# qianlim/CAPE

Hardware: AMD Instinct MI355X
Metric: meshes/sec fwd+bwd, CAPE-affineconv nz64 @ batch 16, 1/2/4/8 MI355X (higher is better)
Workload: dtype f32

## Files before the change

cape_amd/_lib.py:

```python
import ctypes as C
import os

import torch

_HERE = os.path.dirname(os.path.abspath(__file__))
LIB_PATH = os.path.join(_HERE, "libcape_hip.so")

MAX_SRC = 8
ACT = {"none": 0, "leaky": 1, "relu": 2, "tanh": 3}
BIAS_NONE, BIAS_CHANNEL, BIAS_VERTEX = 0, 1, 2


class CapeSrc(C.Structure):
    _fields_ = [
        ("x", C.c_void_p), ("x_sample_stride", C.c_int64), ("ldx", C.c_int32), ("C", C.c_int32),
        ("w", C.c_void_p), ("w_rs", C.c_int64), ("w_cs", C.c_int64),
        ("w2", C.c_void_p), ("w2_rs", C.c_int64), ("w2_cs", C.c_int64),
    ]


class CapeCondLayer(C.Structure):
    _fields_ = [("w", C.c_void_p), ("w_aff", C.c_void_p), ("coef", C.c_void_p), ("dcoef", C.c_void_p),
                ("gw", C.c_void_p), ("gw_aff", C.c_void_p), ("K", C.c_int32), ("F", C.c_int32)]

# ... 68 lines not shown
    "cape_gconv_fwd": (C.c_int, [_SRCP, _i32, _p, _i64, _i32, _i32, _i32, _i32, _p, _i32, _i32, _p,
                                 C.POINTER(CapeRank), _i32, _p]),
    "cape_gconv_fwd_plan": (C.c_int, [_SRCP, _i32, _i32, _i32, _i32, C.POINTER(_i32)]),
    "cape_gconv_fwd_h2": (C.c_int, [_SRCP, _i32, _p, _i64, _i32, _i32, _i32, _i32, _p, _i32, _i32, _p,
                                    C.POINTER(CapeRank), _i32, C.POINTER(CapeH2), _p]),
    "cape_gconv_fwd_plan_h2": (C.c_int, [_SRCP, _i32, _i32, _i32, _i32, C.POINTER(CapeH2), C.POINTER(_i32)]),
    "cape_gconv_dw_stage_h2": (C.c_int, [_SRCP, _i32, _p, _i64, _i32, _p, C.c_uint32, _i32, _i32, _i32, _i32, _p, _i64, _i32,
                                         C.POINTER(CapeH2Dw), _p]),
    "cape_gconv_dw_plan_h2": (C.c_int, [_SRCP, _i32, _p, _i64, _i32, _p, C.c_uint32, _i32, _i32, _i32, C.POINTER(CapeH2Dw),
                                        C.POINTER(_i32)]),
    "cape_rowmax": (C.c_int, [_p, _i64, _i32, _i32, _i32, _i32, _p, _i32, _p]),
    "cape_weight_pieces_blocks": (C.c_int, [C.c_void_p, _i32, C.POINTER(_i32), C.POINTER(_i32)]),
    "cape_weight_pieces": (C.c_int, [_p, _i32, _p, _i32, _p, _i32, _p]),
    "cape_rowscale_reduce_workspace_bytes": (_i64, [_i32, _i32, _i32, _i32]),
    "cape_rowscale_reduce": (C.c_int, [_p, _i64, _i32, _p, _i32, _i32, _i32, _i32, _p, _p, _i64, _p]),
    "cape_gconv_dw_workspace_bytes": (_i64, [_SRCP, _i32, _i32, _i32, _i32]),
    "cape_gconv_dw": (C.c_int, [_SRCP, _i32, _p, _i64, _i32, _p, C.c_uint32, _i32, _i32, _i32, _i32, _p, _i64, _p]),
    "cape_gconv_dw_stage": (C.c_int, [_SRCP, _i32, _p, _i64, _i32, _p, C.c_uint32, _i32, _i32, _i32, _i32, _p, _i64, _i32, _p]),
    "cape_condnet_fwd": (C.c_int, [_p, _i32, _p, _i32, _p, _p, _p, _p, _p, _p, _p, _p, _p, _i32, _i32, _i32, _i32, _i32, _i32, _p]),
    "cape_condnet_bwd": (C.c_int, [_p, _i32, _p, _i32, _p, _p, _p, _i32, _p, _i32, _p, _p, _p, _p, _p, _p, _i32, _i32, _i32, _i32, _i32, _i32, _p]),
    "cape_gconv_dw_reduce_batch": (C.c_int, [C.c_void_p, _i32, _p]),
    "cape_gconv_dw_batch": (C.c_int, [C.c_void_p, _i32, _p]),
    "cape_gconv_dw_batch_plan": (C.c_int, [C.c_void_p, _i32, C.POINTER(_i32), _i32, C.POINTER(_i32)]),
    "cape_gconv_dw_plan": (C.c_int, [_SRCP, _i32, _p, _i64, _i32, _p, C.c_uint32, _i32, _i32, _i32, C.POINTER(_i32)]),
    "cape_gconv_fwd_bf16": (C.c_int, [_SRCP, _i32, _p, _i64, _i32, _i32, _i32, _i32, _p, _i32, _i32, _p,
                                      C.POINTER(CapeRank), _i32, _p]),
    "cape_gconv_fwd_plan_bf16": (C.c_int, [_SRCP, _i32, _i32, _i32, _i32, C.POINTER(_i32)]),
    "cape_gconv_dw_bf16": (C.c_int, [_SRCP, _i32, _p, _i64, _i32, _p, C.c_uint32, _i32, _i32, _i32, _i32, _p, _i64, _p]),
    "cape_gconv_dw_stage_bf16": (C.c_int, [_SRCP, _i32, _p, _i64, _i32, _p, C.c_uint32, _i32, _i32, _i32, _i32, _p, _i64, _i32, _p]),
    "cape_gconv_dw_plan_bf16": (C.c_int, [_SRCP, _i32, _p, _i64, _i32, _p, C.c_uint32, _i32, _i32, _i32, C.POINTER(_i32)]),
    "cape_bwd_prep_workspace_bytes": (_i64, [_i32, _i32, _i32, _i32]),
    "cape_bwd_prep": (C.c_int, [_p, _i64, _i32, _p, _i64, _i32, _i32, _p, _p, _i64, _i32, _p, _p, _i32, _p, _i32, _p,
                                _i64, _i32, _i32, _i32, _i32, _p, _i64, _p, _p]),
    "cape_bwd_prep_plan": (C.c_int, [_p, _i64, _i32, _p, _i64, _i32, _i32, _p, _p, _i64, _i32, _i32, _i32, _i32, _i32, C.POINTER(_i32)]),
    "cape_bwd_prep_finalize": (C.c_int, [C.c_void_p, _i32, _p]),
    "cape_spmm": (C.c_int, [_p, _i64, _i32, _p, _p, _p, _i32, _i32, _f32, _p, _i64, _i32, _f32, _p, _i64, _i32,
                            _i32, _i32, _i32, _p, _p]),
    "cape_spmm_multi": (C.c_int, [C.POINTER(CapeSpmmTerm), _i32, _i32, _p, _i64, _i32, _i32, _i32, _i32, _p, _p]),
    "cape_spmm_multi_actgrad_chunks": (_i32, [_p, _i64, _i32, _p, _i64, _i32, _i32, _i32]),
    "cape_spmm_multi_actgrad": (C.c_int, [C.POINTER(CapeSpmmTerm), _i32, _p, _i64, _i32, _i32, _i32, _i32, _p, _p, _i64, _i32, _i32, _p, _p]),
    "cape_spmm_multi_actgrad_chunks_bf16": (_i32, [_p, _i64, _i32, _p, _i64, _i32, _i32, _i32]),
    "cape_spmm_multi_actgrad_bf16": (C.c_int, [C.POINTER(CapeSpmmTerm), _i32, _p, _i64, _i32, _i32, _i32, _i32, _p, _p, _i64, _i32, _i32, _p, _p]),
    "cape_bwd_prep_spmm_chunks": (_i32, [_p, _i64, _i32, _p, _i64, _i32, _p, _i64, _i32, _i32, _i32, _i32]),
    "cape_spmm_multi_prep_chunks_bf16": (_i32, [C.POINTER(CapeSpmmTerm), _i32, _i32, _i32, _i32]),
    "cape_spmm_multi_prep_bf16": (C.c_int, [C.POINTER(CapeSpmmTerm), _i32, C.c_uint32, _p, _i32, _i32, _i32, _i32, _p, _i64, _p]),
    "cape_bwd_prep_spmm_chunks_bf16": (_i32, [_p, _i64, _i32, _p, _i64, _i32, _p, _i64, _i32, _i32, _i32, _i32]),
# ... 113 lines not shown
```

cape_amd/csrc/gconv.hip:

```cpp
#include "common.h"
#include "gconv_shared.h"
#include "gemm_plain.h"
#include "gemm_split.h"
#include "gemm_h2.h"
#include "narrow.h"
#include <stdlib.h>
#include <algorithm>
#include <vector>

namespace {

constexpr int KC_DEFAULT = 32;

template <int ROWS, int LDA, int KC, typename AT = float>
__device__ __forceinline__ void stage_rows(float *sA, const SrcDev &S, int n, int r0, int Mo,
                                            int c0, int tid) {
    constexpr int QPR = KC / 4;
    constexpr int RP = 256 / QPR;
    const int q = tid % QPR;
    const int rl0 = tid / QPR;
    const int c = c0 + 4 * q;
    const AT *x0 = reinterpret_cast<const AT *>(S.x) + (long long)n * S.xs;
    const AT *xb = x0 + c;
    const int nvalid = S.C - c;
    constexpr int P = ROWS / RP;
    if (S.vec && (nvalid >= 4 || (nvalid > 0 && c + 4 <= S.ldx) || nvalid <= 0)) {
        float4 v[P];
#pragma unroll
        for (int pass = 0; pass < P; ++pass) {
// ... 1086 lines not shown

extern "C" int cape_gconv_dw_reduce_batch(const cape_dw_item_t *items, int32_t nitems, void *stream) {
    if (!items || nitems < 1 || nitems > CAPE_MAX_DW_REDUCE_ITEMS) return CAPE_EINVAL;
    DwReduceBatch B;
    B.n = nitems;
    int off = 0;
    for (int i = 0; i < nitems; ++i) {
        const cape_dw_item_t &t = items[i];
        int blocks = 0;
        const int rc = gconv_dw_stage_impl(t.srcs, t.nsrc, (const float *)t.dz, t.dz_sample_stride, t.lddz, (const float *)t.dz2,
                                           t.dz2_mask, t.N, t.Mo, t.F, t.accumulate, t.workspace, t.workspace_bytes, 3, stream,
                                           t.bf16 != 0, &B.it[i], &B.vec[i], &blocks, t.h2);
        if (rc) return rc;
        B.blk_off[i] = off;
        off += blocks;
    }
    B.blk_off[nitems] = off;
    CAPE_LAUNCH(dw_reduce_batch_kernel, dim3((unsigned)off), dim3(256), 0, (hipStream_t)stream, B);
    CAPE_LAUNCH_CHECK();
    return CAPE_OK;
}

namespace {
struct DwbShape { int N, tiles, nseg, ngroups, rsplit, rows_per_split; };
struct DwbLaunch {
    int first, n;
    int order[DWB_MAX_ITEMS];
    int rot[DWB_MAX_ITEMS];
    int start[8][DWB_MAX_ITEMS + 2];
    int grid, units;
};

inline int dwb_on_xcd(int count, int rot, int x) {
    const int s0 = (x - rot) & 7;
    return s0 < count ? (count - 1 - s0) / 8 + 1 : 0;
}

inline void dwb_plan_launch(const DwbShape *sh, int n, DwbLaunch &L) {
    long long rows[DWB_MAX_ITEMS];
    L.units = 0;
    for (int i = 0; i < n; ++i) {
        L.order[i] = i;
        rows[i] = (long long)(sh[i].N / sh[i].ngroups) * sh[i].rows_per_split;
        L.units += sh[i].tiles * sh[i].ngroups * sh[i].rsplit;
    }
    std::stable_sort(L.order, L.order + n, [&](int a, int b) { return rows[a] > rows[b]; });
    long long load[8] = {0, 0, 0, 0, 0, 0, 0, 0};
    for (int k = 0; k < n; ++k) {
        const int i = L.order[k], count = sh[i].ngroups * sh[i].rsplit;
// ... 3 lines not shown
        for (int r = 0; r < 8; ++r) {
            long long peak = 0;
            for (int x = 0; x < 8; ++x) {
                const long long v = load[x] + w * dwb_on_xcd(count, r, x);
                peak = v > peak ? v : peak;
            }
            if (best_peak < 0 || peak < best_peak) { best_peak = peak; best = r; }
        }
        L.rot[k] = best;
        for (int x = 0; x < 8; ++x) load[x] += w * dwb_on_xcd(count, best, x);
    }
    int longest = 0;
    for (int x = 0; x < 8; ++x) {
        int start = 0;
        for (int k = 0; k < DWB_MAX_ITEMS + 2; ++k) {
            L.start[x][k] = start;
            if (k < n) start += sh[L.order[k]].tiles * dwb_on_xcd(sh[L.order[k]].ngroups * sh[L.order[k]].rsplit, L.rot[k], x);
        }
        longest = start > longest ? start : longest;
    }
    L.grid = 8 * longest;
}

inline void dwb_plan(const DwbShape *sh, int n, std::vector<DwbLaunch> &out) {
    out.clear();
    int i = 0;
    while (i < n) {
        DwbLaunch L;
        L.first = i;
        int segs = 0, k = 0;
        while (i + k < n && k < DWB_MAX_ITEMS && segs + sh[i + k].nseg <= DWB_MAX_SEGS) {
            segs += sh[i + k].nseg;
            ++k;
        }
        L.n = k;
        dwb_plan_launch(sh + i, k, L);
        out.push_back(L);
        i += k;
    }
}

inline int dwb_describe(const cape_dw_item_t &t, DwDescribe &d, DwbShape &s) {
    if (t.bf16 || !t.h2) return CAPE_EINVAL;
    const int rc = gconv_dw_stage_impl(t.srcs, t.nsrc, (const float *)t.dz, t.dz_sample_stride, t.lddz, (const float *)t.dz2,
                                       t.dz2_mask, t.N, t.Mo, t.F, t.accumulate, t.workspace, t.workspace_bytes, 1, nullptr,
                                       false, nullptr, nullptr, nullptr, t.h2, &d);
    if (rc) return rc;
    if (!d.use_h2 || !d.v4 || t.nsrc > DWB_MAX_SEGS) return CAPE_EINVAL;
    s.N = t.N; s.nseg = t.nsrc;
    s.tiles = d.pl.ntiles;
    s.ngroups = d.pl.ngroups; s.rsplit = d.pl.rsplit; s.rows_per_split = d.pl.rows_per_split;
    return CAPE_OK;
}

int dwb_prepare(const cape_dw_item_t *items, int nitems, std::vector<DwDescribe> &desc, std::vector<DwbShape> &sh,
                std::vector<DwbLaunch> &launches) {
    if (!items || nitems < 1 || nitems > CAPE_MAX_DW_REDUCE_ITEMS) return CAPE_EINVAL;
    desc.resize(nitems);
    sh.resize(nitems);
    for (int i = 0; i < nitems; ++i) {
        const int rc = dwb_describe(items[i], desc[i], sh[i]);
        if (rc) return rc;
    }
    dwb_plan(sh.data(), nitems, launches);
    return CAPE_OK;
}
}

extern "C" int cape_gconv_dw_batch_plan(const cape_dw_item_t *items, int32_t nitems, int32_t *units, int32_t max_units, int32_t info[4]) {
    std::vector<DwDescribe> desc;
    std::vector<DwbShape> sh;
    std::vector<DwbLaunch> launches;
    const int rc = dwb_prepare(items, nitems, desc, sh, launches);
    if (rc) return rc;
    if (!info) return CAPE_EINVAL;
    int nunits = 0, grid = 0;
    for (size_t l = 0; l < launches.size(); ++l) {
        const DwbLaunch &L = launches[l];
        grid = L.grid > grid ? L.grid : grid;
        for (int x = 0; x < 8; ++x)
            for (int tk = 0; tk < L.n; ++tk) {
                const int k = L.order[tk];
                const DwDescribe &d = desc[L.first + k];
                const DwbShape &c = sh[L.first + k];
                const int spg = c.N / c.ngroups;
                for (int j = L.start[x][tk]; j < L.start[x][tk + 1]; ++j, ++nunits) {
                    if (!units || nunits >= max_units) continue;
                    const int q = (j - L.start[x][tk]) / c.tiles, t = (j - L.start[x][tk]) % c.tiles;
                    const int split = ((x - L.rot[tk]) & 7) + 8 * q;
                    int si = 0;
                    while (si + 1 < d.p.nsrc && t >= d.p.tile_off[si + 1]) ++si;
                    const int grp = split / c.rsplit, rs = split % c.rsplit;
                    const int wra = rs * c.rows_per_split, rb = wra + c.rows_per_split < d.p.Mo ? wra + c.rows_per_split : d.p.Mo;
                    int32_t *u = units + 10 * (size_t)nunits;
                    u[0] = (int32_t)l; u[1] = 8 * j + x; u[2] = L.first + k; u[3] = si; u[4] = t - d.p.tile_off[si];
                    u[5] = split; u[6] = grp * spg; u[7] = grp * spg + spg; u[8] = wra; u[9] = rb;
                }
            }
    }
    info[0] = (int32_t)launches.size(); info[1] = nunits; info[2] = (int32_t)sizeof(DwParams); info[3] = grid;
    return CAPE_OK;
}

extern "C" int cape_gconv_dw_batch(const cape_dw_item_t *items, int32_t nitems, void *stream) {
    std::vector<DwDescribe> desc;
    std::vector<DwbShape> sh;
    std::vector<DwbLaunch> launches;
    const int rc = dwb_prepare(items, nitems, desc, sh, launches);
    if (rc) return rc;
    for (const DwbLaunch &L : launches) {
        DwParams P = DwParams();
        DwBatch &B = P.bt;
        int seg = 0;
        for (int tk = 0; tk < L.n; ++tk) {
            const int k = L.order[tk];
            const DwParams &p = desc[L.first + k].p;
            DwBatchItem &it = B.item[tk];
            it.dz = p.dz; it.dzrm = p.dzrm; it.dz2 = p.dz2; it.dz2rm = p.dz2rm; it.dzs = p.dzs;
            it.ws = p.ws; it.slab = p.slab;
            it.lddz = p.lddz; it.dzrmw = p.dzrmw; it.dz2rmw = p.dz2rmw; it.F = p.F; it.N = p.N; it.Mo = p.Mo; it.ftiles = p.ftiles;
            it.rsplit = p.rsplit; it.rows_per_split = p.rows_per_split; it.samples_per_group = p.samples_per_group;
            it.seg0 = seg; it.nseg = p.nsrc;
            it.ntiles = sh[L.first + k].tiles; it.rot = L.rot[tk];
            for (int s = 0; s < p.nsrc; ++s, ++seg) {
                DwBatchSeg &sg = B.seg[seg];
                sg.x = p.s[s].x; sg.rm = p.s[s].rm; sg.xs = p.s[s].xs; sg.part_off = p.part_off[s];
                sg.ldx = p.s[s].ldx; sg.C = p.s[s].C;
                sg.rmw_use2 = p.s[s].rmw | (int)((p.dz2_mask >> s) & 1u) << 16;
                sg.tile_off = p.tile_off[s];
            }
        }
        B.nseg = seg;
        for (int x = 0; x < 8; ++x)
            for (int g = 0; g < DWB_MAX_ITEMS + 2; ++g) B.start[x][g] = L.start[x][g];
        if (L.grid < 8) return CAPE_EINVAL;
        CAPE_LAUNCH((dw_h2_kernel<128, 128, true>), dim3((unsigned)L.grid), dim3(256 * H2_DW_KG), 0, (hipStream_t)stream, P);
        CAPE_LAUNCH_CHECK();
    }
    return CAPE_OK;
}
```

cape_amd/csrc/gconv_shared.h:

```cpp
#pragma once
#include "common.h"

namespace {

struct SrcDev {
    const float *x;
    long long xs;
    int ldx, C;
    const float *w;
    long long wrs, wcs;
    const float *w2;
    long long w2rs, w2cs;
    int vec;
    const unsigned short *wh, *wl;
    long long wp;
    const unsigned short *wh2, *wl2;
    long long wp2;
    const float *rm;
    int rmw;
};

struct GconvParams {
    SrcDev s[CAPE_MAX_SRC];
    int nsrc;
// ... 30 lines not shown
__device__ __forceinline__ void h2_store_rowmax(const GconvParams &p, int n, int row0, int cb, const float (&gm)[4], int lane) {
    const int lh = lane >> 5, sel = (lane >> 4) & 1;
    const float m01 = h2_max_pair(gm[0], gm[1]), m23 = h2_max_pair(gm[2], gm[3]);
    if ((lane & 15) == 0) {
        const int nvalid = (p.F + 31) >> 5;
#pragma unroll
        for (int h = 0; h < 2; ++h) {
            const int j = 2 * h + sel;
            const float m = h ? m23 : m01;
#pragma unroll
            for (int i = 0; i < 4; ++i) {
                const int r = row0 + 8 * j + 4 * lh + i;
                if (r < p.Mo) {
                    float *dst = p.rm_out + ((long long)n * p.Mo + r) * p.rm_out_w;
                    dst[cb] = m;
                    if (cb == 0)
                        for (int e = nvalid; e < p.rm_out_w; ++e) dst[e] = 0.f;
                }
            }
        }
    }
}

constexpr int DWB_MAX_ITEMS = 6, DWB_MAX_SEGS = 12;
struct DwBatchItem {
    const float *dz, *dzrm;
    const float *dz2, *dz2rm;
    long long dzs;
    float *ws;
    long long slab;
    int lddz, dzrmw, dz2rmw, F, N, Mo, ftiles;
    int rsplit, rows_per_split, samples_per_group;
    int seg0, nseg;
    int ntiles, rot;
};
struct DwBatchSeg {
    const float *x, *rm;
    long long xs;
    long long part_off;
    int ldx, C;
    int rmw_use2;
    int tile_off;
};
struct DwBatch {
    DwBatchItem item[DWB_MAX_ITEMS];
    DwBatchSeg seg[DWB_MAX_SEGS];
    int start[8][DWB_MAX_ITEMS + 2];
    int nseg = 0;
    int pad_;
};

struct DwParams {
    SrcDev s[CAPE_MAX_SRC];
    int nsrc;
    const float *dz;
    const float *dz2;
    unsigned dz2_mask;
    long long dzs;
    int lddz, dzvec;
    int N, Mo, F;
    int ftiles;
    int tile_off[CAPE_MAX_SRC + 1];
    long long part_off[CAPE_MAX_SRC + 1];
    int rsplit, rows_per_split;
    int ngroups, samples_per_group;
    float *ws;
    long long slab;
    const float *dzrm, *dz2rm;
    int dzrmw, dz2rmw;
    int vstart[CAPE_MAX_SRC + 1];
    DwBatch bt;
};
static_assert(sizeof(DwParams) <= 3584, "kernel arguments: 4 KB including the hidden ones");

template <int BM, int BN, int WAVES_M, int WAVES_N, bool DUAL, typename AT = float>
__device__ __forceinline__ void gconv_epilogue(const GconvParams &p,
                                               f32x16 (&acc)[BM / WAVES_M / 32][BN / WAVES_N / 32],
                                               f32x16 (&acc2)[DUAL ? BM / WAVES_M / 32 : 1][DUAL ? BN / WAVES_N / 32 : 1],
                                               int n, int r0, int f0, int wm, int wn, int li, int lh) {
    constexpr int WTM = BM / WAVES_M, WTN = BN / WAVES_N;
    constexpr int TM = WTM / 32, TN = WTN / 32;
    AT *yb = reinterpret_cast<AT *>(p.y) + (long long)n * p.ys;
#pragma unroll
    for (int a = 0; a < TM; ++a) {
#pragma unroll
        for (int b = 0; b < TN; ++b) {
            const int f = f0 + wn * WTN + b * 32 + li;
            const int fm = p.deintK > 1 ? (f % p.deintK) * p.deint_stride + f / p.deintK : f;
            float coef[CAPE_MAX_SRC];
#pragma unroll
            for (int j = 0; j < CAPE_MAX_SRC; ++j)
                coef[j] = (j < p.rankR && f < p.F) ? p.coef[((long long)n * p.rankR + j) * p.F + f] : 0.f;
            float gm[4] = {0.f, 0.f, 0.f, 0.f};
#pragma unroll
            for (int g = 0; g < 16; ++g) {
                const int r = r0 + wm * WTM + a * 32 + (g & 3) + 8 * (g >> 2) + 4 * lh;
// ... 70 lines not shown
```

cape_amd/csrc/gemm_h2.h:

```cpp
#pragma once
#include <stddef.h>
#include <stdio.h>
#include <stdlib.h>
#include <type_traits>

#include "gconv_shared.h"

namespace {

typedef _Float16 h2_half8 __attribute__((ext_vector_type(8)));
typedef _Float16 h2_half2 __attribute__((ext_vector_type(2)));
typedef unsigned h2_u32x4 __attribute__((ext_vector_type(4)));

constexpr int H2_KC = 32;
constexpr int H2_ROW = 64;

__device__ __forceinline__ unsigned h2_bits(float v) { return __builtin_bit_cast(unsigned, v); }
__device__ __forceinline__ float h2_float(unsigned v) { return __builtin_bit_cast(float, v); }

__device__ __forceinline__ void h2_split2(float x0, float x1, unsigned &hi, unsigned &lo) {
    const _Float16 h0 = (_Float16)x0, h1 = (_Float16)x1;
    const _Float16 l0 = (_Float16)(x0 - (float)h0), l1 = (_Float16)(x1 - (float)h1);
    const h2_half2 H = {h0, h1}, L = {l0, l1};
    hi = __builtin_bit_cast(unsigned, H);
// ... 295 lines not shown
__global__ __launch_bounds__(256 * H2_DW_KG, 1) void dw_h2_kernel(DwParams p) {
    constexpr int RK = 32, KG = H2_DW_KG;
    constexpr int WTM = CT / 2, WTN = FT / 2;
    constexpr int TM = WTM / 32, TN = WTN / 32;
    constexpr int CPA = CT / 64, CPB = FT / 64;
    static_assert(TM >= 1 && TN >= 1 && (CT == 64 || CT == 128) && (FT == 64 || FT == 128), "tile");
    constexpr int ROW = 64, APL2 = CT * ROW, BPL2 = FT * ROW, STAGE2 = 2 * (APL2 + BPL2);
    __shared__ __attribute__((aligned(16))) unsigned char smem_all[KG * 2 * STAGE2];
    __shared__ float red[2][4 * KG];
    static_assert(2 * STAGE2 >= TM * TN * 16 * 256 * 4, "a group's stages hold its accumulator for the final sum");

    const int kg = __builtin_amdgcn_readfirstlane((int)threadIdx.x >> 8);
    const int tid = threadIdx.x & 255, lane = tid & 63, wave = tid >> 6;
    unsigned char *smem = smem_all + kg * 2 * STAGE2;
    const int wm = wave >> 1, wn = wave & 1, li = lane & 31, lh = lane >> 5;
    const int rg = tid >> 6;
    const int ca = tid & 63, fb = tid & 63;

    typedef const __attribute__((address_space(4))) char *KArg;
    const KArg karg = (KArg)__builtin_amdgcn_kernarg_segment_ptr();
    struct { const float *x, *rm; long long xs; int ldx, C, rmw; } S;
    struct { const float *dz, *rmz; float *out; long long dzs; int wz, lddz, F, N, Mo, ftiles, rsplit, rows_per_split, samples_per_group; } W;
    int lt, split;
    constexpr bool CAN_BATCH = CT == 128 && FT == 128 && V4;
    if (CAN_BATCH && p.bt.nseg > 0) {
        const int xcd = (int)blockIdx.x & 7, j = (int)blockIdx.x >> 3;
        typedef const __attribute__((address_space(4))) int *StartTab;
        typedef const __attribute__((address_space(4))) DwBatchSeg *SegTab;
        typedef const __attribute__((address_space(4))) DwBatchItem *ItemTab;
        const StartTab st = (StartTab)(karg + offsetof(DwParams, bt) + offsetof(DwBatch, start)) + xcd * (DWB_MAX_ITEMS + 2);
        const SegTab sgt = (SegTab)(karg + offsetof(DwParams, bt) + offsetof(DwBatch, seg));
        const ItemTab itt = (ItemTab)(karg + offsetof(DwParams, bt) + offsetof(DwBatch, item));
        int ii = 0, j0 = st[0];
#pragma unroll
        for (int i = 1; i < DWB_MAX_ITEMS; ++i) {
            const int o = st[i];
            if (j >= o) { ii = i; j0 = o; }
        }
        if (j >= st[DWB_MAX_ITEMS]) return;
        const int ntl = itt[ii].ntiles;
        const int q = (j - j0) / ntl;
        const int tile = (j - j0) - q * ntl;
        split = ((xcd - itt[ii].rot) & 7) + 8 * q;
        int sg = itt[ii].seg0;
        const int sg_end = sg + itt[ii].nseg;
        while (sg + 1 < sg_end && tile >= sgt[sg + 1].tile_off) ++sg;
        lt = tile - sgt[sg].tile_off;
        S.x = sgt[sg].x; S.rm = sgt[sg].rm; S.xs = sgt[sg].xs; S.ldx = sgt[sg].ldx; S.C = sgt[sg].C;
// ... 430 lines not shown
```

cape_amd/ops.py:

```python
import ctypes as C

import numpy as np
import torch

from . import _lib
from ._lib import lib, CapeSrc, check
from .graph import ConvOperators, HostCSR

import os as _os
FUSED_RECURRENCE = int(_os.environ.get("CAPE_FUSED_RECURRENCE", "1"))
CMR_FUSED_TAIL = int(_os.environ.get("CAPE_CMR_FUSED_TAIL", "1"))
MERGED_D_PASS = _os.environ.get("CAPE_MERGED_D_PASS", "auto")


def merged_d_pass(batch):
    if MERGED_D_PASS == "auto":
        return 2 * int(batch) <= 32
    return bool(int(MERGED_D_PASS))
SPMM_ELL = int(_os.environ.get("CAPE_SPMM_ELL", "1"))

_ACT_OF = {"b1leakyrelu": ("leaky", _lib.BIAS_CHANNEL), "b1relu": ("relu", _lib.BIAS_CHANNEL),
           "b1tanh": ("tanh", _lib.BIAS_CHANNEL), "b2relu": ("relu", _lib.BIAS_VERTEX)}


# ... 254 lines not shown
        return "gemm_h2_kernel<%d, %d, %s>" % (bm, bn, tf(dual))
    if fam == 2:
        return "gemm_split_kernel<%d, %d, %s, %s%s>" % (bm, bn, tf(layout), tf(dual), at)
    if fam == 1:
        return "gemm_plain_kernel<%d, %d, %s, %s, %s>" % (bm, bn, waves, tf(dual), tf(layout))
    return "gconv_fwd_kernel<%d, %d, %s, %s, 32%s>" % (bm, bn, waves, tf(dual), at)


def dw_kernel_name(fam, ct, ft, bf16=False):
    if fam in (5, 6):
        return _DW_FAMILY[fam]
    if fam == 4:
        return "dw_h2_kernel<%d, %d, %s>" % (ct, ft, "true" if (DW_V4 and (ct, ft) == (128, 128)) else "false")
    if fam == 3 or fam == 0:
        return "%s<%d, %d, %s>" % (_DW_FAMILY[fam], ct, ft, "unsigned short" if bf16 else "float")
    waves = "4, 1" if (fam == 2 and ft == 32) else "2, 2"
    return "%s<%d, %d, %s, %s>" % (_DW_FAMILY[fam], ct, ft, waves, "unsigned short" if bf16 else "float")


FUSE_ACT_GRAD = int(_os.environ.get("CAPE_FUSE_ACT_GRAD", "1"))
FUSE_PREP_SPMM = int(_os.environ.get("CAPE_FUSE_PREP_SPMM", "1"))
DW_V4 = int(_os.environ.get("CAPE_DW_V4", "1"))
DW_BATCH = int(_os.environ.get("CAPE_DW_BATCH", "1"))
_CHAIN = [False]


class _ActOffer(object):
    __slots__ = ("act", "gB", "fused")

    def __init__(self, act, gB):
        self.act, self.gB, self.fused = act, gB, False


class sole_consumer_chain(object):
    def __init__(self, on=True):
        self.on = bool(on)

    def __enter__(self):
        self.prev, _CHAIN[0] = _CHAIN[0], self.on
        return self

    def __exit__(self, *exc):
        _CHAIN[0] = self.prev
        return False


# ... 257 lines not shown
    def dw_stage(which):
        if h2 is not None:
            check(lib.cape_gconv_dw_stage_h2(arr, len(entries), p, ss, ld, p2, mask, N, Mo, F, 1 if accumulate else 0,
                                             C.c_void_p(ws.data_ptr()), need, which, C.byref(h2), _stream()), "cape_gconv_dw_stage_h2")
        else:
            check(_fn("cape_gconv_dw_stage", dz)(arr, len(entries), p, ss, ld, p2, mask, N, Mo, F, 1 if accumulate else 0,
                                                 C.c_void_p(ws.data_ptr()), need, which, _stream()), "cape_gconv_dw_stage")

    def launch():
        dw_stage(0)

    if defer and DEFERRED is not None and LAUNCH_LOG is None:
        if PLAN_LOG is not None:
            plan = (C.c_int32 * 4)()
            dw_plan(plan)
            PLAN_LOG.add(("dw", plan[0], plan[1], plan[2]) + (("bf16",) if bf else ()))
        it = _lib.CapeDwItem()
        it.srcs, it.nsrc = C.addressof(arr), len(entries)
        it.dz, it.dz_sample_stride, it.lddz = p.value, ss, ld
        it.dz2, it.dz2_mask = (p2.value if p2 is not None else None), mask
        it.N, it.Mo, it.F, it.accumulate, it.bf16 = N, Mo, F, 1 if accumulate else 0, 1 if bf else 0
        it.workspace, it.workspace_bytes = ws.data_ptr(), need
        it.h2 = C.addressof(h2) if h2 is not None else None
        batch = bool(DW_BATCH) and h2 is not None and \
            lib.cape_gconv_dw_batch_plan(C.addressof(it), 1, None, 0, (C.c_int32 * 4)()) == 0
        if not batch:
            dw_stage(1)
        held = [dz] + ([dz2] if dz2 is not None else []) + [e["x"] for e in entries] + (list(h2._keep) if batch else [])
        vers = [t._version for t in held] if batch else None
        DEFERRED_DW.append((it, arr, ws, held, h2, batch, vers))
        return
    if LAUNCH_LOG is None and PLAN_LOG is None:
        launch()
    else:
        plan = (C.c_int32 * 4)()
        dw_plan(plan)
        fam, ct, ft, nslab = list(plan)
        if PLAN_LOG is not None:
            PLAN_LOG.add(("dw", fam, ct, ft) + (("bf16",) if bf else ()))
        if LAUNCH_LOG is None:
            launch()
            return
        flops, byts = _dw_work(entries, N, Mo, F, bool(mask))
        sumCF = sum(int(e.get("C", e["x"].shape[2])) for e in entries) * F
        _log_launch(dw_kernel_name(fam, ct, ft, bf), flops, byts, lambda: dw_stage(1))
        _log_launch("dw_reduce", 0, 4 * sumCF * (nslab + 1), lambda: dw_stage(2))


# ... 201 lines not shown
    check(rc, "cape_fill_cond")
    return y


def reduce_cond(dy, scale=None, out=None, accumulate=False):
    _lib.require_gpu()
    N, M, Cn = dy.shape
    if out is None:
        out = torch.empty((N, Cn), device=dy.device, dtype=torch.float32)
    gp, gs, gl = _v(dy)
    rc = lib.cape_reduce_cond(gp, gs, gl, _ptr(scale), C.c_void_p(out.data_ptr()), out.stride(0) if N > 1 else Cn,
                              N, M, Cn, 1 if accumulate else 0, _stream())
    check(rc, "cape_reduce_cond")
    return out


NO_WEIGHT_GRAD = None


DEFERRED = None
DEFERRED_DW = []
DEFERRED_GN = []

def _flush_dw():
    if DEFERRED_DW:
        queued, DEFERRED_DW[:] = list(DEFERRED_DW), []
        nmax = 12
        bat = [i for i, q in enumerate(queued) if q[5]]
        for i in bat:
            held, vers = queued[i][3], queued[i][6]
            if any(t._version != v for t, v in zip(held, vers)):
                raise RuntimeError("an operand of a deferred weight gradient (dz, dz2, a source or its row bounds) was written in "
                                   "place between gconv_dw(defer=True) and flush_deferred(): the batched contraction reads it at "
                                   "the flush (CAPE_DW_BATCH=0 contracts at once)")
        for i0 in range(0, len(bat), nmax):
            idx = bat[i0:i0 + nmax]
            arr = (_lib.CapeDwItem * len(idx))(*[queued[i][0] for i in idx])
            check(lib.cape_gconv_dw_batch(C.addressof(arr), len(idx), _stream()), "cape_gconv_dw_batch")
        for i0 in range(0, len(queued), nmax):
            chunk = queued[i0:i0 + nmax]
            arr = (_lib.CapeDwItem * len(chunk))(*[q[0] for q in chunk])
            check(lib.cape_gconv_dw_reduce_batch(C.addressof(arr), len(chunk), _stream()), "cape_gconv_dw_reduce_batch")


def flush_deferred():
    global DEFERRED
    if DEFERRED_GN:
        queued, DEFERRED_GN[:] = list(DEFERRED_GN), []
        nmax = 32
        for i0 in range(0, len(queued), nmax):
            chunk = queued[i0:i0 + nmax]
            arr = (_lib.CapeGnParamItem * len(chunk))()
            for a, (dgb, dst_g, dst_b) in zip(arr, chunk):
                a.dgamma_partial, a.dbeta_partial = dgb[0].data_ptr(), dgb[1].data_ptr()
                a.dgamma, a.dbeta = dst_g.data_ptr(), dst_b.data_ptr()
                a.N, a.C = int(dgb.shape[1]), int(dgb.shape[2])
            check(lib.cape_groupnorm_param_reduce_batch(C.addressof(arr), len(chunk), _stream()), "cape_groupnorm_param_reduce_batch")
    _flush_dw()
    if not DEFERRED:
        return
    items, DEFERRED[:] = list(DEFERRED), []
    _finalize_bwd_prep(items)


def _finalize_bwd_prep(items):
    for i0 in range(0, len(items), 16):
        chunk = items[i0:i0 + 16]
        arr = (_lib.CapeBwdPrepItem * len(chunk))()
        for a, it in zip(arr, chunk):
            a.workspace = it["ws"].data_ptr()
            a.N, a.Mo, a.F, a.R = it["N"], it["Mo"], it["F"], it["R"]
            a.dbias = None if it["dbias"] is None else it["dbias"].data_ptr()
            a.dcoef = None if it["dcoef"] is None else it["dcoef"].data_ptr()
            a.dcoef_g = None if it["dcoef_g"] is None else it["dcoef_g"].data_ptr()
            a.dcoef_sample_stride = it["cstride"]
            a.chunks = int(it.get("chunks", 0))
        check(lib.cape_bwd_prep_finalize(arr, len(chunk), _stream()), "cape_bwd_prep_finalize")


def _alloc_dcoef(N, R, F, dev, want_g, joint):
    if joint and R and want_g:
        dcoef = torch.empty((N, R + 1, F), device=dev, dtype=torch.float32)
        return dcoef, dcoef[:, R], (R + 1) * F
    dcoef = torch.empty((N, R, F), device=dev, dtype=torch.float32) if R else None
    dcoef_g = torch.empty((N, F), device=dev, dtype=torch.float32) if want_g else None
# ... 1058 lines not shown
                assert gW.shape == W.shape and gW.is_contiguous() and (Wa is None or (gWa.shape == Wa.shape and gWa.is_contiguous()))
                d.gw = gW.data_ptr() + 4 * Ch * K * F
                d.gw_aff = None if Wa is None else gWa.data_ptr() + 4 * Ch * F
        return arr

    @staticmethod
    def forward(ctx, cond, layers):
        _lib.require_gpu()
        cond = cond.contiguous()
        N, Cc = cond.shape
        coefs = []
        for ly in layers:
            W, Wa, K = ly["W"], ly["Wa"], int(ly["K"])
            assert W.is_contiguous() and W.shape[0] == (int(ly["Ch"]) + Cc) * K and (Wa is None or Wa.is_contiguous())
            coefs.append(torch.empty((N, K + (0 if Wa is None else 1), W.shape[1]), device=cond.device, dtype=torch.float32))
        arr = CondCoefFn._descr(layers, N, coefs=coefs)
        check(lib.cape_cond_coef_fwd(C.c_void_p(cond.data_ptr()), Cc, N, Cc, arr, len(layers), _stream()), "cape_cond_coef_fwd")
        ctx.layers = layers
        ctx.save_for_backward(cond)
        return tuple(coefs)

    @staticmethod
    def backward(ctx, *dcoefs):
        flush_deferred()
        (cond,) = ctx.saved_tensors
        layers = ctx.layers
        N, Cc = cond.shape
        dcoefs = [torch.zeros((N, int(ly["K"]) + (0 if ly["Wa"] is None else 1), ly["W"].shape[1]), device=cond.device)
                  if d is None else d.contiguous() for d, ly in zip(dcoefs, layers)]
        arr = CondCoefFn._descr(layers, N, dcoefs=dcoefs, grads=True)
        dcond = torch.empty_like(cond) if ctx.needs_input_grad[0] else None
        check(lib.cape_cond_coef_bwd(C.c_void_p(cond.data_ptr()), Cc, N, Cc, arr, len(layers), _ptr(dcond), Cc, 0, _stream()),
              "cape_cond_coef_bwd")
        return dcond, None


class CondNetsFn(torch.autograd.Function):

    @staticmethod
    def forward(ctx, c1, c2, W1, b1, W2, b2, Wc, bc, gbufs, copies=1):
        _lib.require_gpu()
        c1, c2 = c1.contiguous(), c2.contiguous()
        N, in1 = c1.shape
        hid, out1, in2, out2 = int(W1.shape[1]), int(W2.shape[1]), int(c2.shape[1]), int(Wc.shape[1])
        assert all(t.is_contiguous() and t.dtype == torch.float32 for t in (W1, b1, W2, b2, Wc, bc, c1, c2))
        assert tuple(W1.shape) == (in1, hid) and tuple(W2.shape) == (hid, out1) and tuple(Wc.shape) == (in2, out2)
        h = torch.empty((N, hid), device=c1.device, dtype=torch.float32)
# ... 398 lines not shown
```

include/cape_hip.h:

```cpp
#ifndef CAPE_HIP_H
#define CAPE_HIP_H

#include <stdint.h>

#ifdef __cplusplus
extern "C" {
#endif

#define CAPE_ABI_VERSION 18
#define CAPE_MAX_SRC 8

#define CAPE_OK 0
#define CAPE_EINVAL (-1)
#define CAPE_EUNSORTED (-2)
#define CAPE_ERANGE (-3)
#define CAPE_EWORKSPACE (-4)

#define CAPE_ACT_NONE 0
#define CAPE_ACT_LEAKY 1
#define CAPE_ACT_RELU 2
#define CAPE_ACT_TANH 3

#define CAPE_BIAS_NONE 0
#define CAPE_BIAS_CHANNEL 1
// ... 113 lines not shown
                           int64_t workspace_bytes, int32_t stage, const cape_h2_dw_t *h2, void *stream);
int cape_gconv_dw_plan_h2(const cape_src_t *srcs, int32_t nsrc, const float *dz, int64_t dz_sample_stride, int32_t lddz,
                          const float *dz2, uint32_t dz2_mask, int32_t N, int32_t Mo, int32_t F, const cape_h2_dw_t *h2,
                          int32_t plan[4]);

#define CAPE_MAX_DW_REDUCE_ITEMS 12
typedef struct cape_dw_item {
    const cape_src_t *srcs;
    int32_t nsrc;
    const void *dz;
    int64_t dz_sample_stride;
    int32_t lddz;
    const void *dz2;
    uint32_t dz2_mask;
    int32_t N, Mo, F, accumulate, bf16;
    void *workspace;
    int64_t workspace_bytes;
    const struct cape_h2_dw *h2;
} cape_dw_item_t;
int cape_gconv_dw_reduce_batch(const cape_dw_item_t *items, int32_t nitems, void *stream);

int cape_gconv_dw_batch(const cape_dw_item_t *items, int32_t nitems, void *stream);
int cape_gconv_dw_batch_plan(const cape_dw_item_t *items, int32_t nitems, int32_t *units, int32_t max_units, int32_t info[4]);

int cape_gconv_dw_plan(const cape_src_t *srcs, int32_t nsrc, const float *dz, int64_t dz_sample_stride, int32_t lddz,
                       const float *dz2, uint32_t dz2_mask, int32_t N, int32_t Mo, int32_t F, int32_t plan[4]);

int64_t cape_bwd_prep_workspace_bytes(int32_t N, int32_t Mo, int32_t F, int32_t R);
int cape_bwd_prep(const float *g, int64_t g_sample_stride, int32_t ldg, const float *y,
                  int64_t y_sample_stride, int32_t ldy, int32_t act, const uint32_t *mask, float *dz,
                  int64_t dz_sample_stride, int32_t lddz, float *dbias, const float *rowscale,
                  int32_t R, float *dcoef, int32_t rg, float *dcoef_g, int64_t dcoef_sample_stride, int32_t finalize,
                  int32_t N, int32_t Mo, int32_t F, void *workspace, int64_t workspace_bytes, float *rowmax_out, void *stream);

#define CAPE_BP_GENERIC 0
#define CAPE_BP_NARROW 1
#define CAPE_BP_VEC4 2
#define CAPE_BP_VEC8 3
#define CAPE_BP_BOUND_NONE 0
#define CAPE_BP_BOUND_KERNEL 1
#define CAPE_BP_BOUND_STANDALONE 2
int cape_bwd_prep_plan(const float *g, int64_t g_sample_stride, int32_t ldg, const float *y, int64_t y_sample_stride,
                       int32_t ldy, int32_t act, const uint32_t *mask, const float *dz, int64_t dz_sample_stride, int32_t lddz,
                       int32_t N, int32_t Mo, int32_t F, int32_t want_rowmax, int32_t plan[6]);

#define CAPE_MAX_BWD_PREP_ITEMS 16
// ... 319 lines not shown
```

Baseline: 6360.

## Sweep deferred weight-gradient contractions across all tile variants in fewer batched launches

Adds a sweep mode that groups all deferred weight-gradient items (up to 64) by kernel tile variant, not only the 128x128 v4 variant, and packs up to 10 items and 24 segments per launch. DwParams now overlays the single-item fields and the batch table in a union so the larger batch still fits the kernel-argument limit. Condnet backward flushes only the pending bwd-prep finals, which keeps weight gradients deferred longer so more of them land in one sweep. The aim is fewer kernel launches and better load spread across XCDs, at the cost of host-side planning work and a bigger argument block.

```diff
diff --git a/cape_amd/_lib.py b/cape_amd/_lib.py
--- a/cape_amd/_lib.py
+++ b/cape_amd/_lib.py
@@ -114,6 +114,8 @@
     "cape_gconv_dw_reduce_batch": (C.c_int, [C.c_void_p, _i32, _p]),
     "cape_gconv_dw_batch": (C.c_int, [C.c_void_p, _i32, _p]),
     "cape_gconv_dw_batch_plan": (C.c_int, [C.c_void_p, _i32, C.POINTER(_i32), _i32, C.POINTER(_i32)]),
+    "cape_gconv_dw_sweep": (C.c_int, [C.c_void_p, _i32, _p]),
+    "cape_gconv_dw_sweep_plan": (C.c_int, [C.c_void_p, _i32, C.POINTER(_i32), _i32, C.POINTER(_i32)]),
     "cape_gconv_dw_plan": (C.c_int, [_SRCP, _i32, _p, _i64, _i32, _p, C.c_uint32, _i32, _i32, _i32, C.POINTER(_i32)]),
     "cape_gconv_fwd_bf16": (C.c_int, [_SRCP, _i32, _p, _i64, _i32, _i32, _i32, _i32, _p, _i32, _i32, _p,
                                       C.POINTER(CapeRank), _i32, _p]),
diff --git a/cape_amd/csrc/gconv.hip b/cape_amd/csrc/gconv.hip
--- a/cape_amd/csrc/gconv.hip
+++ b/cape_amd/csrc/gconv.hip
@@ -5,6 +5,7 @@
 #include "gemm_h2.h"
 #include "narrow.h"
 #include <stdlib.h>
+#include <string.h>
 #include <algorithm>
 #include <vector>
 
@@ -1137,9 +1138,11 @@
 }
 
 namespace {
-struct DwbShape { int N, tiles, nseg, ngroups, rsplit, rows_per_split; };
+struct DwbShape { int N, tiles, nseg, ngroups, rsplit, rows_per_split, kernel; };
 struct DwbLaunch {
-    int first, n;
+    int n;
+    int idx[DWB_MAX_ITEMS];
+    int kernel;
     int order[DWB_MAX_ITEMS];
     int rot[DWB_MAX_ITEMS];
     int start[8][DWB_MAX_ITEMS + 2];
@@ -1189,57 +1192,83 @@
     L.grid = 8 * longest;
 }
 
-inline void dwb_plan(const DwbShape *sh, int n, std::vector<DwbLaunch> &out) {
-    out.clear();
-    int i = 0;
-    while (i < n) {
+inline int dwb_kernel_of(bool v4, int ct, int ft) { return v4 ? 4 : 2 * (ct == 128) + (ft == 128); }
+
+inline void dwb_plan(const DwbShape *sh, const std::vector<int> &members, int max_items, int max_segs, std::vector<DwbLaunch> &out) {
+    size_t i = 0;
+    while (i < members.size()) {
         DwbLaunch L;
-        L.first = i;
+        DwbShape loc[DWB_MAX_ITEMS];
         int segs = 0, k = 0;
-        while (i + k < n && k < DWB_MAX_ITEMS && segs + sh[i + k].nseg <= DWB_MAX_SEGS) {
-            segs += sh[i + k].nseg;
+        while (i + k < members.size() && k < max_items && segs + sh[members[i + k]].nseg <= max_segs) {
+            loc[k] = sh[members[i + k]];
+            L.idx[k] = members[i + k];
+            segs += loc[k].nseg;
             ++k;
         }
         L.n = k;
-        dwb_plan_launch(sh + i, k, L);
+        L.kernel = loc[0].kernel;
+        dwb_plan_launch(loc, k, L);
         out.push_back(L);
         i += k;
     }
 }
 
-inline int dwb_describe(const cape_dw_item_t &t, DwDescribe &d, DwbShape &s) {
+inline int dwb_describe(const cape_dw_item_t &t, DwDescribe &d, DwbShape &s, bool any_kernel) {
     if (t.bf16 || !t.h2) return CAPE_EINVAL;
     const int rc = gconv_dw_stage_impl(t.srcs, t.nsrc, (const float *)t.dz, t.dz_sample_stride, t.lddz, (const float *)t.dz2,
                                        t.dz2_mask, t.N, t.Mo, t.F, t.accumulate, t.workspace, t.workspace_bytes, 1, nullptr,
                                        false, nullptr, nullptr, nullptr, t.h2, &d);
     if (rc) return rc;
-    if (!d.use_h2 || !d.v4 || t.nsrc > DWB_MAX_SEGS) return CAPE_EINVAL;
+    if (!d.use_h2 || (!d.v4 && !any_kernel) || t.nsrc > DWB_BATCH_SEGS) return CAPE_EINVAL;
     s.N = t.N; s.nseg = t.nsrc;
     s.tiles = d.pl.ntiles;
     s.ngroups = d.pl.ngroups; s.rsplit = d.pl.rsplit; s.rows_per_split = d.pl.rows_per_split;
+    s.kernel = dwb_kernel_of(d.v4, d.pl.ct, d.pl.ft);
     return CAPE_OK;
 }
 
-int dwb_prepare(const cape_dw_item_t *items, int nitems, std::vector<DwDescribe> &desc, std::vector<DwbShape> &sh,
-                std::vector<DwbLaunch> &launches) {
-    if (!items || nitems < 1 || nitems > CAPE_MAX_DW_REDUCE_ITEMS) return CAPE_EINVAL;
+int dwb_prepare(const cape_dw_item_t *items, int nitems, bool sweep, std::vector<DwDescribe> &desc, std::vector<DwbShape> &sh,
+                std::vector<DwbLaunch> &launches, int *refused) {
+    if (refused) *refused = -1;
+    if (!items || nitems < 1 || nitems > (sweep ? CAPE_MAX_DW_SWEEP_ITEMS : CAPE_MAX_DW_REDUCE_ITEMS)) return CAPE_EINVAL;
     desc.resize(nitems);
     sh.resize(nitems);
     for (int i = 0; i < nitems; ++i) {
-        const int rc = dwb_describe(items[i], desc[i], sh[i]);
-        if (rc) return rc;
-    }
-    dwb_plan(sh.data(), nitems, launches);
+        const int rc = dwb_describe(items[i], desc[i], sh[i], sweep);
+        if (rc) {
+            if (refused) *refused = i;
+            return rc;
+        }
+    }
+    launches.clear();
+    std::vector<int> members;
+    if (!sweep) {
+        for (int i = 0; i < nitems; ++i) members.push_back(i);
+        dwb_plan(sh.data(), members, DWB_BATCH_ITEMS, DWB_BATCH_SEGS, launches);
+        return CAPE_OK;
+    }
+    std::vector<char> taken(nitems, 0);
+    for (int i = 0; i < nitems; ++i) {
+        if (taken[i]) continue;
+        members.clear();
+        for (int k = i; k < nitems; ++k)
+            if (!taken[k] && sh[k].kernel == sh[i].kernel) { members.push_back(k); taken[k] = 1; }
+        dwb_plan(sh.data(), members, DWB_MAX_ITEMS, DWB_MAX_SEGS, launches);
+    }
     return CAPE_OK;
 }
-}
-
-extern "C" int cape_gconv_dw_batch_plan(const cape_dw_item_t *items, int32_t nitems, int32_t *units, int32_t max_units, int32_t info[4]) {
+
+int dwb_plan_query(const cape_dw_item_t *items, int32_t nitems, bool sweep, int32_t *units, int32_t max_units, int32_t info[4]) {
     std::vector<DwDescribe> desc;
     std::vector<DwbShape> sh;
     std::vector<DwbLaunch> launches;
-    const int rc = dwb_prepare(items, nitems, desc, sh, launches);
-    if (rc) return rc;
+    int refused = -1;
+    const int rc = dwb_prepare(items, nitems, sweep, desc, sh, launches, &refused);
+    if (rc) {
+        if (sweep && info && refused >= 0) { info[0] = refused; info[1] = info[2] = info[3] = 0; }
+        return rc;
+    }
     if (!info) return CAPE_EINVAL;
     int nunits = 0, grid = 0;
     for (size_t l = 0; l < launches.size(); ++l) {
@@ -1248,8 +1277,8 @@
         for (int x = 0; x < 8; ++x)
             for (int tk = 0; tk < L.n; ++tk) {
                 const int k = L.order[tk];
-                const DwDescribe &d = desc[L.first + k];
-                const DwbShape &c = sh[L.first + k];
+                const DwDescribe &d = desc[L.idx[k]];
+                const DwbShape &c = sh[L.idx[k]];
                 const int spg = c.N / c.ngroups;
                 for (int j = L.start[x][tk]; j < L.start[x][tk + 1]; ++j, ++nunits) {
                     if (!units || nunits >= max_units) continue;
@@ -1260,7 +1289,7 @@
                     const int grp = split / c.rsplit, rs = split % c.rsplit;
                     const int wra = rs * c.rows_per_split, rb = wra + c.rows_per_split < d.p.Mo ? wra + c.rows_per_split : d.p.Mo;
                     int32_t *u = units + 10 * (size_t)nunits;
-                    u[0] = (int32_t)l; u[1] = 8 * j + x; u[2] = L.first + k; u[3] = si; u[4] = t - d.p.tile_off[si];
+                    u[0] = (int32_t)l; u[1] = 8 * j + x; u[2] = L.idx[k]; u[3] = si; u[4] = t - d.p.tile_off[si];
                     u[5] = split; u[6] = grp * spg; u[7] = grp * spg + spg; u[8] = wra; u[9] = rb;
                 }
             }
@@ -1269,27 +1298,29 @@
     return CAPE_OK;
 }
 
-extern "C" int cape_gconv_dw_batch(const cape_dw_item_t *items, int32_t nitems, void *stream) {
+int dwb_run(const cape_dw_item_t *items, int32_t nitems, bool sweep, void *stream) {
     std::vector<DwDescribe> desc;
     std::vector<DwbShape> sh;
     std::vector<DwbLaunch> launches;
-    const int rc = dwb_prepare(items, nitems, desc, sh, launches);
+    const int rc = dwb_prepare(items, nitems, sweep, desc, sh, launches, nullptr);
     if (rc) return rc;
     for (const DwbLaunch &L : launches) {
         DwParams P = DwParams();
+        memset(&P.bt, 0, sizeof(P.bt));
         DwBatch &B = P.bt;
         int seg = 0;
         for (int tk = 0; tk < L.n; ++tk) {
             const int k = L.order[tk];
-            const DwParams &p = desc[L.first + k].p;
+            const DwParams &p = desc[L.idx[k]].p;
             DwBatchItem &it = B.item[tk];
             it.dz = p.dz; it.dzrm = p.dzrm; it.dz2 = p.dz2; it.dz2rm = p.dz2rm; it.dzs = p.dzs;
             it.ws = p.ws; it.slab = p.slab;
             it.lddz = p.lddz; it.dzrmw = p.dzrmw; it.dz2rmw = p.dz2rmw; it.F = p.F; it.N = p.N; it.Mo = p.Mo; it.ftiles = p.ftiles;
             it.rsplit = p.rsplit; it.rows_per_split = p.rows_per_split; it.samples_per_group = p.samples_per_group;
             it.seg0 = seg; it.nseg = p.nsrc;
-            it.ntiles = sh[L.first + k].tiles; it.rot = L.rot[tk];
+            it.ntiles = sh[L.idx[k]].tiles; it.rot = L.rot[tk];
             for (int s = 0; s < p.nsrc; ++s, ++seg) {
+                if (seg >= DWB_MAX_SEGS) return CAPE_EINVAL;
                 DwBatchSeg &sg = B.seg[seg];
                 sg.x = p.s[s].x; sg.rm = p.s[s].rm; sg.xs = p.s[s].xs; sg.part_off = p.part_off[s];
                 sg.ldx = p.s[s].ldx; sg.C = p.s[s].C;
@@ -1297,12 +1328,37 @@
                 sg.tile_off = p.tile_off[s];
             }
         }
-        B.nseg = seg;
+        P.bt_nseg = seg;
         for (int x = 0; x < 8; ++x)
             for (int g = 0; g < DWB_MAX_ITEMS + 2; ++g) B.start[x][g] = L.start[x][g];
         if (L.grid < 8) return CAPE_EINVAL;
-        CAPE_LAUNCH((dw_h2_kernel<128, 128, true>), dim3((unsigned)L.grid), dim3(256 * H2_DW_KG), 0, (hipStream_t)stream, P);
+        const dim3 grid((unsigned)L.grid), block(256 * H2_DW_KG);
+        hipStream_t st = (hipStream_t)stream;
+        switch (L.kernel) {
+        case 4: CAPE_LAUNCH((dw_h2_kernel<128, 128, true>), grid, block, 0, st, P); break;
+        case 3: CAPE_LAUNCH((dw_h2_kernel<128, 128, false>), grid, block, 0, st, P); break;
+        case 2: CAPE_LAUNCH((dw_h2_kernel<128, 64, false>), grid, block, 0, st, P); break;
+        case 1: CAPE_LAUNCH((dw_h2_kernel<64, 128, false>), grid, block, 0, st, P); break;
+        default: CAPE_LAUNCH((dw_h2_kernel<64, 64, false>), grid, block, 0, st, P); break;
+        }
         CAPE_LAUNCH_CHECK();
     }
     return CAPE_OK;
 }
+}
+
+extern "C" int cape_gconv_dw_batch_plan(const cape_dw_item_t *items, int32_t nitems, int32_t *units, int32_t max_units, int32_t info[4]) {
+    return dwb_plan_query(items, nitems, false, units, max_units, info);
+}
+
+extern "C" int cape_gconv_dw_batch(const cape_dw_item_t *items, int32_t nitems, void *stream) {
+    return dwb_run(items, nitems, false, stream);
+}
+
+extern "C" int cape_gconv_dw_sweep_plan(const cape_dw_item_t *items, int32_t nitems, int32_t *units, int32_t max_units, int32_t info[4]) {
+    return dwb_plan_query(items, nitems, true, units, max_units, info);
+}
+
+extern "C" int cape_gconv_dw_sweep(const cape_dw_item_t *items, int32_t nitems, void *stream) {
+    return dwb_run(items, nitems, true, stream);
+}
diff --git a/cape_amd/csrc/gconv_shared.h b/cape_amd/csrc/gconv_shared.h
--- a/cape_amd/csrc/gconv_shared.h
+++ b/cape_amd/csrc/gconv_shared.h
@@ -1,5 +1,6 @@
 #pragma once
 #include "common.h"
+#include <type_traits>
 
 namespace {
 
@@ -76,7 +77,8 @@
     }
 }
 
-constexpr int DWB_MAX_ITEMS = 6, DWB_MAX_SEGS = 12;
+constexpr int DWB_MAX_ITEMS = 10, DWB_MAX_SEGS = 24;
+constexpr int DWB_BATCH_ITEMS = 6, DWB_BATCH_SEGS = 12;
 struct DwBatchItem {
     const float *dz, *dzrm;
     const float *dz2, *dz2rm;
@@ -100,32 +102,37 @@
     DwBatchItem item[DWB_MAX_ITEMS];
     DwBatchSeg seg[DWB_MAX_SEGS];
     int start[8][DWB_MAX_ITEMS + 2];
-    int nseg = 0;
-    int pad_;
 };
 
 struct DwParams {
-    SrcDev s[CAPE_MAX_SRC];
-    int nsrc;
-    const float *dz;
-    const float *dz2;
-    unsigned dz2_mask;
-    long long dzs;
-    int lddz, dzvec;
-    int N, Mo, F;
-    int ftiles;
-    int tile_off[CAPE_MAX_SRC + 1];
-    long long part_off[CAPE_MAX_SRC + 1];
-    int rsplit, rows_per_split;
-    int ngroups, samples_per_group;
-    float *ws;
-    long long slab;
-    const float *dzrm, *dz2rm;
-    int dzrmw, dz2rmw;
-    int vstart[CAPE_MAX_SRC + 1];
-    DwBatch bt;
+    union {
+        struct {
+            SrcDev s[CAPE_MAX_SRC];
+            int nsrc;
+            const float *dz;
+            const float *dz2;
+            unsigned dz2_mask;
+            long long dzs;
+            int lddz, dzvec;
+            int N, Mo, F;
+            int ftiles;
+            int tile_off[CAPE_MAX_SRC + 1];
+            long long part_off[CAPE_MAX_SRC + 1];
+            int rsplit, rows_per_split;
+            int ngroups, samples_per_group;
+            float *ws;
+            long long slab;
+            const float *dzrm, *dz2rm;
+            int dzrmw, dz2rmw;
+            int vstart[CAPE_MAX_SRC + 1];
+        };
+        DwBatch bt;
+    };
+    int bt_nseg = 0;
+    int pad_ = 0;
 };
 static_assert(sizeof(DwParams) <= 3584, "kernel arguments: 4 KB including the hidden ones");
+static_assert(std::is_trivially_copyable<DwBatch>::value && std::is_trivially_copyable<DwParams>::value, "the halves travel as bytes");
 
 template <int BM, int BN, int WAVES_M, int WAVES_N, bool DUAL, typename AT = float>
 __device__ __forceinline__ void gconv_epilogue(const GconvParams &p,
diff --git a/cape_amd/csrc/gemm_h2.h b/cape_amd/csrc/gemm_h2.h
--- a/cape_amd/csrc/gemm_h2.h
+++ b/cape_amd/csrc/gemm_h2.h
@@ -341,8 +341,7 @@
     struct { const float *x, *rm; long long xs; int ldx, C, rmw; } S;
     struct { const float *dz, *rmz; float *out; long long dzs; int wz, lddz, F, N, Mo, ftiles, rsplit, rows_per_split, samples_per_group; } W;
     int lt, split;
-    constexpr bool CAN_BATCH = CT == 128 && FT == 128 && V4;
-    if (CAN_BATCH && p.bt.nseg > 0) {
+    if (p.bt_nseg > 0) {
         const int xcd = (int)blockIdx.x & 7, j = (int)blockIdx.x >> 3;
         typedef const __attribute__((address_space(4))) int *StartTab;
         typedef const __attribute__((address_space(4))) DwBatchSeg *SegTab;
diff --git a/cape_amd/ops.py b/cape_amd/ops.py
--- a/cape_amd/ops.py
+++ b/cape_amd/ops.py
@@ -300,6 +300,8 @@
 FUSE_PREP_SPMM = int(_os.environ.get("CAPE_FUSE_PREP_SPMM", "1"))
 DW_V4 = int(_os.environ.get("CAPE_DW_V4", "1"))
 DW_BATCH = int(_os.environ.get("CAPE_DW_BATCH", "1"))
+DW_SWEEP = int(_os.environ.get("CAPE_DW_SWEEP", "1"))
+DW_SWEEP_LOG = None
 _CHAIN = [False]
 
 
@@ -603,8 +605,8 @@
         it.N, it.Mo, it.F, it.accumulate, it.bf16 = N, Mo, F, 1 if accumulate else 0, 1 if bf else 0
         it.workspace, it.workspace_bytes = ws.data_ptr(), need
         it.h2 = C.addressof(h2) if h2 is not None else None
-        batch = bool(DW_BATCH) and h2 is not None and \
-            lib.cape_gconv_dw_batch_plan(C.addressof(it), 1, None, 0, (C.c_int32 * 4)()) == 0
+        may_wait = lib.cape_gconv_dw_sweep_plan if DW_SWEEP == 2 else lib.cape_gconv_dw_batch_plan
+        batch = bool(DW_BATCH) and h2 is not None and may_wait(C.addressof(it), 1, None, 0, (C.c_int32 * 4)()) == 0
         if not batch:
             dw_stage(1)
         held = [dz] + ([dz2] if dz2 is not None else []) + [e["x"] for e in entries] + (list(h2._keep) if batch else [])
@@ -852,6 +854,24 @@
 DEFERRED_DW = []
 DEFERRED_GN = []
 
+def _dw_launches(arr, n):
+    query = lib.cape_gconv_dw_sweep_plan if DW_SWEEP else lib.cape_gconv_dw_batch_plan
+    info = (C.c_int32 * 4)()
+    check(query(C.addressof(arr), n, None, 0, info), "dw plan query")
+    units = (C.c_int32 * (10 * info[1]))()
+    check(query(C.addressof(arr), n, units, info[1], info), "dw plan query")
+    members = [set() for _ in range(info[0])]
+    for u in range(info[1]):
+        members[units[10 * u]].add(units[10 * u + 2])
+    out = []
+    for m in members:
+        it, plan = arr[min(m)], (C.c_int32 * 4)()
+        check(lib.cape_gconv_dw_plan_h2(C.cast(it.srcs, _lib._SRCP), it.nsrc, it.dz, it.dz_sample_stride, it.lddz, it.dz2, it.dz2_mask,
+                                        it.N, it.Mo, it.F, C.cast(it.h2, C.POINTER(_lib.CapeH2Dw)), plan), "cape_gconv_dw_plan_h2")
+        out.append((plan[1], plan[2], len(m)))
+    return out
+
+
 def _flush_dw():
     if DEFERRED_DW:
         queued, DEFERRED_DW[:] = list(DEFERRED_DW), []
@@ -863,10 +883,16 @@
                 raise RuntimeError("an operand of a deferred weight gradient (dz, dz2, a source or its row bounds) was written in "
                                    "place between gconv_dw(defer=True) and flush_deferred(): the batched contraction reads it at "
                                    "the flush (CAPE_DW_BATCH=0 contracts at once)")
-        for i0 in range(0, len(bat), nmax):
-            idx = bat[i0:i0 + nmax]
+        nbat = 64 if DW_SWEEP else nmax
+        for i0 in range(0, len(bat), nbat):
+            idx = bat[i0:i0 + nbat]
             arr = (_lib.CapeDwItem * len(idx))(*[queued[i][0] for i in idx])
-            check(lib.cape_gconv_dw_batch(C.addressof(arr), len(idx), _stream()), "cape_gconv_dw_batch")
+            if DW_SWEEP_LOG is not None:
+                DW_SWEEP_LOG.extend(_dw_launches(arr, len(idx)))
+            if DW_SWEEP:
+                check(lib.cape_gconv_dw_sweep(C.addressof(arr), len(idx), _stream()), "cape_gconv_dw_sweep")
+            else:
+                check(lib.cape_gconv_dw_batch(C.addressof(arr), len(idx), _stream()), "cape_gconv_dw_batch")
         for i0 in range(0, len(queued), nmax):
             chunk = queued[i0:i0 + nmax]
             arr = (_lib.CapeDwItem * len(chunk))(*[q[0] for q in chunk])
@@ -891,6 +917,15 @@
         return
     items, DEFERRED[:] = list(DEFERRED), []
     _finalize_bwd_prep(items)
+
+
+def flush_finals():
+    if not DW_SWEEP:
+        flush_deferred()
+        return
+    if DEFERRED:
+        items, DEFERRED[:] = list(DEFERRED), []
+        _finalize_bwd_prep(items)
 
 
 def _finalize_bwd_prep(items):
@@ -1995,7 +2030,7 @@
 
     @staticmethod
     def backward(ctx, *dcoefs):
-        flush_deferred()
+        flush_finals()
         (cond,) = ctx.saved_tensors
         layers = ctx.layers
         N, Cc = cond.shape
diff --git a/include/cape_hip.h b/include/cape_hip.h
--- a/include/cape_hip.h
+++ b/include/cape_hip.h
@@ -159,6 +159,10 @@
 
 int cape_gconv_dw_batch(const cape_dw_item_t *items, int32_t nitems, void *stream);
 int cape_gconv_dw_batch_plan(const cape_dw_item_t *items, int32_t nitems, int32_t *units, int32_t max_units, int32_t info[4]);
+
+#define CAPE_MAX_DW_SWEEP_ITEMS 64
+int cape_gconv_dw_sweep(const cape_dw_item_t *items, int32_t nitems, void *stream);
+int cape_gconv_dw_sweep_plan(const cape_dw_item_t *items, int32_t nitems, int32_t *units, int32_t max_units, int32_t info[4]);
 
 int cape_gconv_dw_plan(const cape_src_t *srcs, int32_t nsrc, const float *dz, int64_t dz_sample_stride, int32_t lddz,
                        const float *dz2, uint32_t dz2_mask, int32_t N, int32_t Mo, int32_t F, int32_t plan[4]);
```

New measurement: 6403, median of 6. About the same (+0.7%).
